# jts/nanopolish

Measured on NVIDIA H100. Metric: hmm_scored_events_per_sec, higher is better.
Workload: dtype f32

## Files before the change

nanopolish_b200/csrc/hmm_forward.cu:

```cuda
#include "hmm_forward_kernel.cuh"
#include <algorithm>
#include <cmath>
#include <vector>

using namespace nph_fwd;

namespace {

__global__ void read_prologue_kernel(const DevRead* __restrict__ reads, const double* __restrict__ drift,
                                     const float* __restrict__ ev_mean, const double* __restrict__ ev_time,
                                     float* __restrict__ level, uint32_t n_reads)
{
    for (uint32_t r = blockIdx.x; r < n_reads; r += gridDim.x) {
        const DevRead rd = reads[r];
        const double dr = drift[r];
        const float* m = ev_mean + rd.event_off;
        const double* t = ev_time + rd.event_off;
        float* out = level + rd.event_off;
        const double t0 = t[0];
        for (uint32_t i = threadIdx.x; i < rd.n_events; i += blockDim.x) {
            const float time = (float)__dsub_rn(t[i], t0);
            out[i] = (float)__dsub_rn((double)m[i], __dmul_rn((double)time, dr));
        }
    }
}

}

static void scratch_layout(const nph_ctx* ctx, NphArena& a, float4** params, float** edge)
{
    const size_t warps = (size_t)ctx->sm_count * kMaxWarpsPerCta;
    for (int si = 0; si < nph_ctx::kSideStreams; ++si) nph_wave_scratch(a, ctx->max_kpad, ctx->max_period, warps, &params[si], &edge[si]);
}

size_t nph_hmm_scratch_bytes(const nph_ctx* ctx)
{
    float4* params[nph_ctx::kSideStreams];
    float* edge[nph_ctx::kSideStreams];
    return nph_layout_bytes([&](NphArena& a) { scratch_layout(ctx, a, params, edge); });
}

int nph_launch_read_prologue(nph_ctx* ctx)
{
    const uint32_t n = (uint32_t)ctx->n_reads;
    if (n == 0) return NPH_OK;
    int grid = (int)std::min<size_t>(n, (size_t)ctx->sm_count * 16);
    read_prologue_kernel<<<grid, 256, 0, ctx->stream>>>(ctx->d_reads.p, ctx->d_drift.p, ctx->d_ev_mean.p,
                                                        ctx->d_ev_time.p, ctx->d_level.p, n);
    NPH_CUDA(ctx, cudaGetLastError());
    return NPH_OK;
}

int nph_launch_hmm_forward(nph_ctx* ctx, float* scores_dev)
{
    FwdParams p{};
    p.level = ctx->d_level.p;
    p.reads = ctx->d_reads.p;
    p.trans = ctx->d_trans.p;
    p.models = ctx->d_models.p;
    p.ranks = ctx->d_ranks.p;
    p.jobs = ctx->d_jobs.p;
    p.logsum_g = ctx->d_logsum.p;
    p.flank = ctx->d_flank.p;
    p.scores = scores_dev ? scores_dev : ctx->d_scores.p;
    p.kpad_stride = ctx->max_kpad;
    p.edge_stride = nph_edge_stride(ctx->max_period);
    p.c = ctx->consts;
    p.lsum_bias = NPH_LOGSUM_SAT_ADDR_BIAS;
    p.lsum_scale = 4u;
    p.progress = (ctx->levels_inflight && ctx->level_chunk_events) ? ctx->d_progress.p : nullptr;
    p.chunk_events = (uint32_t)ctx->level_chunk_events;
    float4* params[nph_ctx::kSideStreams];
    float* edge[nph_ctx::kSideStreams];
    NphArena scratch{ctx->d_scratch.p};
    scratch_layout(ctx, scratch, params, edge);

    NPH_CUDA(ctx, cudaMemsetAsync(ctx->d_counters.p, 0, sizeof(unsigned int) * NPH_NUM_COUNTERS, ctx->stream));
    NPH_CUDA(ctx, cudaEventRecord(ctx->ev0, ctx->stream));
    NPH_CUDA(ctx, cudaEventRecord(ctx->ev_fork, ctx->stream));
    std::vector<size_t> idx;
    for (size_t ci = 0; ci < ctx->classes.size(); ++ci) if (ctx->classes[ci].count) idx.push_back(ci);
    std::sort(idx.begin(), idx.end(), [&](size_t a, size_t b) { return ctx->classes[a].cost > ctx->classes[b].cost; });
    bool used[nph_ctx::kSideStreams] = {false, false, false, false};
    int launches = 0;
    for (size_t t = 0; t < idx.size(); ++t) {
        const size_t ci = idx[t];
        const auto& cl = ctx->classes[ci];
        const int si = (int)(t % nph_ctx::kSideStreams);
        cudaStream_t st = ctx->side[si];
        if (!used[si]) { NPH_CUDA(ctx, cudaStreamWaitEvent(st, ctx->ev_fork, 0)); used[si] = true; }
        p.scratch_params = params[si];
        p.scratch_edge = edge[si];
        int rc = NPH_ERR_STATE;
        switch (cl.group_width) {
            case 4: rc = launch_width<4, false>(ctx, p, cl, (int)ci, st); break;
            case 8: rc = launch_width<8, false>(ctx, p, cl, (int)ci, st); break;
            case 16: rc = launch_width<16, false>(ctx, p, cl, (int)ci, st); break;
            case 32: rc = cl.chained ? launch_width<32, true>(ctx, p, cl, (int)ci, st) : launch_width<32, false>(ctx, p, cl, (int)ci, st); break;
        }
        if (rc != NPH_OK) return rc;
        ++launches;
    }
    for (int si = 0; si < nph_ctx::kSideStreams; ++si) {
        if (!used[si]) continue;
        NPH_CUDA(ctx, cudaEventRecord(ctx->ev_join[si], ctx->side[si]));
        NPH_CUDA(ctx, cudaStreamWaitEvent(ctx->stream, ctx->ev_join[si], 0));
    }
    NPH_CUDA(ctx, cudaEventRecord(ctx->ev1, ctx->stream));
    nph_timing_events(ctx, launches);
    return NPH_OK;
}
```

nanopolish_b200/csrc/hmm_forward_kernel.cuh:

```cuda
#pragma once
#include "hmm_wavefront.cuh"
#include "exact_math.cuh"
#include <climits>

namespace nph_fwd {

static_assert(NPH_TBL_SMEM == NPH_LOGSUM_TBL_LEN, "the shared table must cover every index lsum_sat can form");

constexpr int kMaxWarpsPerCta = 24;
template <int C, int W> struct CtaShape { static constexpr int warps = (W == 32) ? 16 : (C <= 4 ? 24 : (C <= 6 ? 20 : 16)); };
constexpr unsigned kFull = 0xffffffffu;

struct FwdParams {
    const float* level;
    const DevRead* reads;
    const float2* trans;
    const DevModelView* models;
    const uint32_t* ranks;
    const nph_hmm_job* jobs;
    const uint32_t* order;
    uint32_t n_jobs;
    unsigned int* counter;
    const float* logsum_g;
    const float* flank;
    float* scores;
    float4* scratch_params;
    float* scratch_edge;
    uint32_t kpad_stride;
    uint32_t edge_stride;
    uint32_t lsum_bias;
    uint32_t lsum_scale;
    const uint32_t* progress;
    uint32_t chunk_events;
    HmmConsts c;
};

template <int C, int W, bool CHAIN>
__global__ void __launch_bounds__(CtaShape<C, W>::warps * 32, 1) hmm_forward_kernel(const FwdParams p)
{
    static_assert(W == 4 || W == 8 || W == 16 || W == 32, "group width");
    static_assert(!CHAIN || W == 32, "only full-warp groups chain strips");
    constexpr int G = 32 / W;
    constexpr int kWarpsPerCta = CtaShape<C, W>::warps;
    constexpr int kCtaThreads = kWarpsPerCta * 32;
    constexpr int STRIP = W * C;
    extern __shared__ float s_tbl[];
    for (int i = threadIdx.x; i < NPH_TBL_SMEM; i += kCtaThreads) s_tbl[i] = p.logsum_g[i];
    __syncthreads();
    const LogsumTable tb = make_logsum_table(s_tbl, p.lsum_bias, p.lsum_scale);

    const int lane = threadIdx.x & 31;
    const int gl = lane & (W - 1);
    const int grp = lane / W;
    const int warp_global = blockIdx.x * kWarpsPerCta + (threadIdx.x >> 5);
    float4* const my_params = warp_params(p.scratch_params, p.kpad_stride, warp_global) + (W < 32 ? grp * STRIP : 0);
    const EdgeRows edge = warp_edge_rows(p.scratch_edge, p.edge_stride, warp_global);

    const float NEG = -CUDART_INF_F;
    const float lp_mk = p.c.lp_mk, lp_mb = p.c.lp_mb, lp_bb = p.c.lp_bb, lp3 = p.c.lp_bk;
    const float lp_kk = p.c.lp_kk, lp_km = p.c.lp_km;

    for (;;) {
        const uint32_t base = nph_warp_pop(p.counter, (unsigned)G, lane);
        if (base >= p.n_jobs) break;
        const uint32_t slot = base + grp;
        const bool has_job = slot < p.n_jobs;
        const uint32_t job_idx = p.order[has_job ? slot : base];
        const nph_hmm_job job = p.jobs[job_idx];
        const DevRead rd = p.reads[job.read];
        const float2 tr = p.trans[job.read];
        const float lp_mm_self = tr.x, lp_mm_next = tr.y;
        const DevModelView mv = p.models[job.model_id];
        if (p.progress) {
            uint32_t need = has_job ? (uint32_t)((rd.event_off + rd.n_events - 1) / p.chunk_events) + 1u : 0u;
            need = __reduce_max_sync(kFull, need);
            if (lane == 0) {
                const volatile uint32_t* pr = p.progress;
                while (*pr < need) __nanosleep(500);
            }
            __syncwarp();
        }

        const nph_wave_geom geo = nph_wave_geometry((int)job.n_kmers, has_job ? nph_job_events(job) : 0, C, W, CHAIN);
        const int K = geo.K, E = geo.E, stride = job.stride, n_strips = geo.n_strips, P = geo.P;
        const bool pre_clip = (job.flags & NPH_HAF_ALLOW_PRE_CLIP) != 0;
        const bool post_clip = (job.flags & NPH_HAF_ALLOW_POST_CLIP) != 0;

        if (has_job) fill_job_gaussians<W>(my_params, mv, rd, p.ranks + job.rank_off, K, geo.kpad, gl, p.c.log_inv_sqrt_2pi);
        __syncwarp();

        const float* lv = p.level + rd.event_off;
        const long long e_first = (long long)job.event_start;
        const int last_strip = geo.last_strip(), end_lane = geo.end_lane(), end_slot = geo.end_slot();
        const int my_steps = has_job ? geo.total_steps() : 0;
        const int total_steps = (W == 32) ? my_steps : __reduce_max_sync(kFull, my_steps);
        const bool any_pre_clip = __any_sync(kFull, pre_clip);

        float mu[C], sd[C], cc[C], ry[C];
        float Mp[C], Bp[C], Kp[C], Tp[C];
#pragma unroll
        for (int c = 0; c < C; ++c) { mu[c] = 0.f; sd[c] = 1.f; cc[c] = 0.f; ry[c] = 1.f; Mp[c] = NEG; Bp[c] = NEG; Kp[c] = NEG; Tp[c] = NEG; }
        if (!CHAIN && gl * C < K) load_columns<C>(my_params, gl * C, mu, sd, cc, ry);
        float Lm_prev = NEG, Lt_prev = NEG, Lk_prev = NEG;
        float lp_end = NEG;
        int r = 1 - gl;
        int s = 0;
        float x_next = 0.f;
        if (r == 1 && E >= 1) x_next = lv[e_first];
        float em_next = NEG, et_next = NEG, ek_next = NEG;
        const long long x_step = (long long)stride * (long long)sizeof(float);
        unsigned long long x_addr = (unsigned long long)(lv + e_first) + (unsigned long long)((long long)r * x_step);
        const int end_row = (gl == end_lane) ? (post_clip ? 1 : E) : INT_MAX;

        for (int g = 0; g < total_steps; ++g) {
            float Lm = __shfl_up_sync(kFull, Mp[C - 1], 1, W);
            float Lt = __shfl_up_sync(kFull, Tp[C - 1], 1, W);
            float Lk = __shfl_up_sync(kFull, Kp[C - 1], 1, W);
            if (gl == 0) { Lm = CHAIN ? em_next : NEG; Lt = CHAIN ? et_next : NEG; Lk = CHAIN ? ek_next : NEG; }

            const bool in_strip = (r >= 1) && (!CHAIN || s < n_strips);
            const int col0 = (CHAIN ? s * STRIP : 0) + gl * C;
            const bool live = in_strip && (r <= E) && (col0 < K);
            const float x = x_next;

            if (CHAIN && in_strip && r == 1) {
#pragma unroll
                for (int c = 0; c < C; ++c) { Mp[c] = NEG; Bp[c] = NEG; Kp[c] = NEG; Tp[c] = NEG; }
                Lm_prev = NEG; Lt_prev = NEG; Lk_prev = NEG;
                if (col0 < K) load_columns<C>(my_params, col0, mu, sd, cc, ry);
            }
            {
                int rn = r + 1, sn = s;
                if (CHAIN && rn > P) { rn = 1; sn = s + 1; }
                if (rn >= 1 && rn <= E && (!CHAIN || sn < n_strips)) {
                    x_next = CHAIN ? lv[e_first + (long long)(rn - 1) * stride] : __ldca(reinterpret_cast<const float*>(x_addr));
                    if (CHAIN && gl == 0 && sn > 0) { em_next = edge.a[rn]; et_next = edge.b[rn]; ek_next = edge.c[rn]; }
                }
            }

            if (live) {
                const bool do_end = (!CHAIN || s == last_strip) && r >= end_row;

                float lm_prev = Lm_prev, lt_prev = Lt_prev, lk_prev = Lk_prev;
                float lm_cur = Lm, lt_cur = Lt, lk_cur = Lk;
                auto cell = [&](const int c, const bool with_soft) {
                    const float em = log_gauss(x, mu[c], sd[c], cc[c], ry[c]);
                    float m = __fadd_rn(lp_mm_self, Mp[c]);
                    m = lsum_sat(m, __fadd_rn(lp_mm_next, lm_prev), tb);
                    m = lsum_sat(m, Tp[c], tb);
                    m = lsum_sat(m, lt_prev, tb);
                    m = lsum_sat(m, __fadd_rn(lp_km, lk_prev), tb);
                    if (with_soft) m = lsum_sat(m, (col0 == 0 && (r == 1 || pre_clip)) ? p.flank[r - 1] : NEG, tb);
                    m = __fadd_rn(m, em);
                    const float b = lsum_sat(__fadd_rn(lp_mb, Mp[c]), __fadd_rn(lp_bb, Bp[c]), tb);
                    float kk = lsum_sat(__fadd_rn(lp_mk, lm_cur), lt_cur, tb);
                    kk = lsum_sat(kk, __fadd_rn(lp_kk, lk_cur), tb);
                    const float t = __fadd_rn(lp3, b);

                    lm_prev = Mp[c]; lt_prev = Tp[c]; lk_prev = Kp[c];
                    lm_cur = m; lt_cur = t; lk_cur = kk;
                    Mp[c] = m; Bp[c] = b; Kp[c] = kk; Tp[c] = t;
                };
                if (any_pre_clip || g == 0) cell(0, true);
                else cell(0, false);
#pragma unroll
                for (int c = 1; c < C; ++c) cell(c, false);
                Lm_prev = Lm; Lt_prev = Lt; Lk_prev = Lk;

                if (do_end) {
                    float Me = Mp[0], Be = Bp[0], Ke = Kp[0];
#pragma unroll
                    for (int c = 1; c < C; ++c) if (c == end_slot) { Me = Mp[c]; Be = Bp[c]; Ke = Kp[c]; }
                    const float post = p.flank[E - r];
                    lp_end = lsum_sat(lp_end, __fadd_rn(Me, post), tb);
                    lp_end = lsum_sat(lp_end, __fadd_rn(Be, post), tb);
                    lp_end = lsum_sat(lp_end, __fadd_rn(Ke, post), tb);
                }
                if (CHAIN && gl == W - 1 && s < last_strip) { edge.a[r] = Mp[C - 1]; edge.b[r] = Tp[C - 1]; edge.c[r] = Kp[C - 1]; }
            }

            r += 1;
            if (!CHAIN) x_addr += x_step;
            if (CHAIN && r > P) { r = 1; s += 1; }
            if (CHAIN && n_strips > 1) __syncwarp();
        }

        const float result = __shfl_sync(kFull, lp_end, (lane & ~(W - 1)) + end_lane);
        if (gl == 0 && has_job) p.scores[job_idx] = result;
        __syncwarp();
    }
}

template <int C, int W, bool CHAIN>
int launch_class(nph_ctx* ctx, const FwdParams& base, const nph_ctx::ClassLaunch& cl, int class_idx, cudaStream_t stream)
{
    FwdParams p = base;
    p.order = ctx->d_order.p + cl.first;
    p.n_jobs = (uint32_t)cl.count;
    p.counter = ctx->d_counters.p + class_idx;
    const size_t smem = sizeof(float) * NPH_TBL_SMEM;
    NPH_CUDA(ctx, cudaFuncSetAttribute(hmm_forward_kernel<C, W, CHAIN>, cudaFuncAttributeMaxDynamicSharedMemorySize, (int)smem));
    constexpr int kWarpsPerCta = CtaShape<C, W>::warps;
    int grid = ctx->sm_count;
    const size_t warps_needed = (cl.count + (32 / W) - 1) / (32 / W);
    if ((size_t)grid * kWarpsPerCta > warps_needed) grid = (int)((warps_needed + kWarpsPerCta - 1) / kWarpsPerCta);
    if (grid < 1) grid = 1;
    hmm_forward_kernel<C, W, CHAIN><<<grid, kWarpsPerCta * 32, smem, stream>>>(p);
    NPH_CUDA(ctx, cudaGetLastError());
    return NPH_OK;
}

template <int W, bool CHAIN> int launch_width(nph_ctx* ctx, const FwdParams& base, const nph_ctx::ClassLaunch& cl, int class_idx, cudaStream_t stream);

#define NPH_DEFINE_LAUNCH_WIDTH(W, CHAIN)                                                                              \
    template <> int launch_width<W, CHAIN>(nph_ctx * ctx, const FwdParams& base, const nph_ctx::ClassLaunch& cl, int class_idx, cudaStream_t stream) \
    {                                                                                                           \
        switch (cl.cols_per_lane) {                                                                             \
            case 1: return launch_class<1, W, CHAIN>(ctx, base, cl, class_idx, stream);                                       \
            case 2: return launch_class<2, W, CHAIN>(ctx, base, cl, class_idx, stream);                                       \
            case 3: return launch_class<3, W, CHAIN>(ctx, base, cl, class_idx, stream);                                       \
            case 4: return launch_class<4, W, CHAIN>(ctx, base, cl, class_idx, stream);                                       \
            case 5: return launch_class<5, W, CHAIN>(ctx, base, cl, class_idx, stream);                                       \
            case 6: return launch_class<6, W, CHAIN>(ctx, base, cl, class_idx, stream);                                       \
            case 7: return launch_class<7, W, CHAIN>(ctx, base, cl, class_idx, stream);                                       \
            case 8: return launch_class<8, W, CHAIN>(ctx, base, cl, class_idx, stream);                                       \
            case 9: return launch_class<9, W, CHAIN>(ctx, base, cl, class_idx, stream);                                       \
            case 10: return launch_class<10, W, CHAIN>(ctx, base, cl, class_idx, stream);                                     \
        }                                                                                                       \
        return NPH_ERR_STATE;                                                                                   \
    }

}
```

Measured before the change: 1.296 billion.

## Stream consecutive full-warp jobs through one wavefront to hide fill and drain

Adds a streaming path for full-warp, non-chained groups. When a job has more than 32 events and no clipping, the warp runs the jobs it pops back to back through a single skewed wavefront, so the next job's fill diagonal overlaps the previous job's drain. Per-warp job descriptors are double-buffered in shared memory and Gaussian parameters in two scratch lines, which is why the params stride grows. The aim is to remove the idle lanes during each job's ramp-up and ramp-down. In exchange the kernel gains complexity, register pressure and more shared and scratch memory.

```diff
diff --git a/nanopolish_b200/csrc/hmm_forward.cu b/nanopolish_b200/csrc/hmm_forward.cu
--- a/nanopolish_b200/csrc/hmm_forward.cu
+++ b/nanopolish_b200/csrc/hmm_forward.cu
@@ -27,10 +27,12 @@
 
 }
 
+static uint32_t params_stride(const nph_ctx* ctx) { return ctx->max_kpad + 32 * NPH_MAX_COLS; }
+
 static void scratch_layout(const nph_ctx* ctx, NphArena& a, float4** params, float** edge)
 {
     const size_t warps = (size_t)ctx->sm_count * kMaxWarpsPerCta;
-    for (int si = 0; si < nph_ctx::kSideStreams; ++si) nph_wave_scratch(a, ctx->max_kpad, ctx->max_period, warps, &params[si], &edge[si]);
+    for (int si = 0; si < nph_ctx::kSideStreams; ++si) nph_wave_scratch(a, params_stride(ctx), ctx->max_period, warps, &params[si], &edge[si]);
 }
 
 size_t nph_hmm_scratch_bytes(const nph_ctx* ctx)
@@ -63,7 +65,7 @@
     p.logsum_g = ctx->d_logsum.p;
     p.flank = ctx->d_flank.p;
     p.scores = scores_dev ? scores_dev : ctx->d_scores.p;
-    p.kpad_stride = ctx->max_kpad;
+    p.kpad_stride = params_stride(ctx);
     p.edge_stride = nph_edge_stride(ctx->max_period);
     p.c = ctx->consts;
     p.lsum_bias = NPH_LOGSUM_SAT_ADDR_BIAS;
diff --git a/nanopolish_b200/csrc/hmm_forward_kernel.cuh b/nanopolish_b200/csrc/hmm_forward_kernel.cuh
--- a/nanopolish_b200/csrc/hmm_forward_kernel.cuh
+++ b/nanopolish_b200/csrc/hmm_forward_kernel.cuh
@@ -35,6 +35,184 @@
     HmmConsts c;
 };
 
+template <int C, class SoftFn>
+__device__ __forceinline__ void row_update(const float x, const float (&mu)[C], const float (&sd)[C], const float (&cc)[C], const float (&ry)[C],
+                                           float (&Mp)[C], float (&Bp)[C], float (&Kp)[C], float (&Tp)[C],
+                                           float lm_prev, float lt_prev, float lk_prev, float lm_cur, float lt_cur, float lk_cur,
+                                           const float lp_mm_self, const float lp_mm_next, const HmmConsts& k, const bool with_soft, const SoftFn& soft,
+                                           const LogsumTable& tb)
+{
+    auto cell = [&](const int c, const bool fold_soft) {
+        const float em = log_gauss(x, mu[c], sd[c], cc[c], ry[c]);
+        float m = __fadd_rn(lp_mm_self, Mp[c]);
+        m = lsum_sat(m, __fadd_rn(lp_mm_next, lm_prev), tb);
+        m = lsum_sat(m, Tp[c], tb);
+        m = lsum_sat(m, lt_prev, tb);
+        m = lsum_sat(m, __fadd_rn(k.lp_km, lk_prev), tb);
+        if (fold_soft) m = lsum_sat(m, soft(), tb);
+        m = __fadd_rn(m, em);
+        const float b = lsum_sat(__fadd_rn(k.lp_mb, Mp[c]), __fadd_rn(k.lp_bb, Bp[c]), tb);
+        float kk = lsum_sat(__fadd_rn(k.lp_mk, lm_cur), lt_cur, tb);
+        kk = lsum_sat(kk, __fadd_rn(k.lp_kk, lk_cur), tb);
+        const float t = __fadd_rn(k.lp_bk, b);
+
+        lm_prev = Mp[c]; lt_prev = Tp[c]; lk_prev = Kp[c];
+        lm_cur = m; lt_cur = t; lk_cur = kk;
+        Mp[c] = m; Bp[c] = b; Kp[c] = kk; Tp[c] = t;
+    };
+    if (with_soft) cell(0, true);
+    else cell(0, false);
+#pragma unroll
+    for (int c = 1; c < C; ++c) cell(c, false);
+}
+
+template <int C>
+__device__ __forceinline__ float end_fold(float lp_end, const float (&Mp)[C], const float (&Bp)[C], const float (&Kp)[C], const int end_slot, const float post,
+                                          const LogsumTable& tb)
+{
+    float Me = Mp[0], Be = Bp[0], Ke = Kp[0];
+#pragma unroll
+    for (int c = 1; c < C; ++c) if (c == end_slot) { Me = Mp[c]; Be = Bp[c]; Ke = Kp[c]; }
+    lp_end = lsum_sat(lp_end, __fadd_rn(Me, post), tb);
+    lp_end = lsum_sat(lp_end, __fadd_rn(Be, post), tb);
+    return lsum_sat(lp_end, __fadd_rn(Ke, post), tb);
+}
+
+struct JobIn { nph_hmm_job job; DevRead rd; float2 tr; DevModelView mv; };
+__device__ __forceinline__ JobIn fetch_job(const FwdParams& p, const uint32_t job_idx, const bool has_job, const int lane)
+{
+    JobIn j;
+    j.job = p.jobs[job_idx];
+    j.rd = p.reads[j.job.read];
+    j.tr = p.trans[j.job.read];
+    j.mv = p.models[j.job.model_id];
+    if (p.progress) {
+        uint32_t need = has_job ? (uint32_t)((j.rd.event_off + j.rd.n_events - 1) / p.chunk_events) + 1u : 0u;
+        need = __reduce_max_sync(kFull, need);
+        if (lane == 0) {
+            const volatile uint32_t* pr = p.progress;
+            while (*pr < need) __nanosleep(500);
+        }
+        __syncwarp();
+    }
+    return j;
+}
+
+__device__ __forceinline__ bool streams(const nph_hmm_job& job, const int E)
+{
+    return E > 32 && (job.flags & (NPH_HAF_ALLOW_PRE_CLIP | NPH_HAF_ALLOW_POST_CLIP)) == 0;
+}
+
+struct StreamJob {
+    unsigned long long x_addr;
+    uint32_t idx;
+    int E, end_lane, end_slot;
+    float lp_mm_self, lp_mm_next;
+    int x_step;
+};
+
+template <int C>
+__device__ __forceinline__ int stream_job(const FwdParams& p, float4* params, const uint32_t job_idx, const JobIn& j, const int lane, StreamJob* s)
+{
+    const nph_wave_geom geo = nph_wave_geometry((int)j.job.n_kmers, nph_job_events(j.job), C, 32, false);
+    if (lane == 0) {
+        s->x_addr = (unsigned long long)(p.level + j.rd.event_off + j.job.event_start);
+        s->idx = job_idx;
+        s->E = geo.E; s->end_lane = geo.end_lane(); s->end_slot = geo.end_slot();
+        s->lp_mm_self = j.tr.x; s->lp_mm_next = j.tr.y;
+        s->x_step = j.job.stride * (int)sizeof(float);
+    }
+    fill_job_gaussians<32>(params, j.mv, j.rd, p.ranks + j.job.rank_off, geo.K, geo.kpad, lane, p.c.log_inv_sqrt_2pi);
+    return geo.E;
+}
+
+template <int C>
+__device__ uint32_t run_stream(const FwdParams& p, const LogsumTable& tb, const HmmConsts& k, float4* params, int lane, const uint32_t job_idx,
+                               const JobIn& first)
+{
+    asm volatile("" : "+l"(params), "+r"(lane));
+    __shared__ StreamJob s_jobs[CtaShape<C, 32>::warps][2];
+    volatile StreamJob* const sj = s_jobs[threadIdx.x >> 5];
+    auto line = [&](const int i) { return params + (i & 1) * (32 * C); };
+    int n = 0;
+    int E = stream_job<C>(p, line(0), job_idx, first, lane, const_cast<StreamJob*>(&sj[0]));
+
+    const float NEG = -CUDART_INF_F;
+    float mu[C], sd[C], cc[C], ry[C];
+    float Mp[C], Bp[C], Kp[C], Tp[C];
+#pragma unroll
+    for (int c = 0; c < C; ++c) { mu[c] = 0.f; sd[c] = 1.f; cc[c] = 0.f; ry[c] = 1.f; Mp[c] = NEG; Bp[c] = NEG; Kp[c] = NEG; Tp[c] = NEG; }
+    float Lm_prev = NEG, Lt_prev = NEG, Lk_prev = NEG;
+    float lp_mm_self = 0.f, lp_mm_next = 0.f;
+    unsigned long long x_addr = 0;
+    int x_step = 0;
+    float x_next = 0.f;
+    bool has_a = false, has_b = true;
+    uint32_t ended_by = p.n_jobs;
+    __syncwarp();
+    for (;;) {
+        volatile StreamJob& a = sj[(n + 1) & 1];
+        volatile StreamJob& b = sj[n & 1];
+        const int window = has_b ? 33 : a.end_lane + 1;
+        for (int t = 0; t < window; ++t) {
+            float Lm = __shfl_up_sync(kFull, Mp[C - 1], 1);
+            float Lt = __shfl_up_sync(kFull, Tp[C - 1], 1);
+            float Lk = __shfl_up_sync(kFull, Kp[C - 1], 1);
+            if (lane == 0) { Lm = NEG; Lt = NEG; Lk = NEG; }
+            const float x = x_next;
+            if (has_b && t == lane + 1) {
+#pragma unroll
+                for (int c = 0; c < C; ++c) { Mp[c] = NEG; Bp[c] = NEG; Kp[c] = NEG; Tp[c] = NEG; }
+                Lm_prev = NEG; Lt_prev = NEG; Lk_prev = NEG;
+                load_columns<C>(line(n), lane * C, mu, sd, cc, ry);
+                lp_mm_self = b.lp_mm_self; lp_mm_next = b.lp_mm_next;
+            }
+            if (t == lane) { x_addr = b.x_addr; x_step = b.x_step; }
+            if (t < lane ? has_a : has_b) {
+                x_next = __ldca(reinterpret_cast<const float*>(x_addr));
+                x_addr += x_step;
+            }
+            if (t <= lane ? has_a : has_b) {
+                row_update<C>(x, mu, sd, cc, ry, Mp, Bp, Kp, Tp, Lm_prev, Lt_prev, Lk_prev, Lm, Lt, Lk, lp_mm_self, lp_mm_next, k, true,
+                              [&] { return (lane == 0 && t == 1) ? p.flank[0] : NEG; }, tb);
+                Lm_prev = Lm; Lt_prev = Lt; Lk_prev = Lk;
+                if (t == lane && lane == a.end_lane) p.scores[a.idx] = end_fold<C>(NEG, Mp, Bp, Kp, a.end_slot, p.flank[0], tb);
+            }
+        }
+        if (!has_b) break;
+
+#pragma unroll 1
+        for (int g = E - 33; g > 0; --g) {
+            float Lm = __shfl_up_sync(kFull, Mp[C - 1], 1);
+            float Lt = __shfl_up_sync(kFull, Tp[C - 1], 1);
+            float Lk = __shfl_up_sync(kFull, Kp[C - 1], 1);
+            if (lane == 0) { Lm = NEG; Lt = NEG; Lk = NEG; }
+            const float x = x_next;
+            x_next = __ldca(reinterpret_cast<const float*>(x_addr));
+            x_addr += x_step;
+            row_update<C>(x, mu, sd, cc, ry, Mp, Bp, Kp, Tp, Lm_prev, Lt_prev, Lk_prev, Lm, Lt, Lk, lp_mm_self, lp_mm_next, k, false,
+                          [&] { return NEG; }, tb);
+            Lm_prev = Lm; Lt_prev = Lt; Lk_prev = Lk;
+        }
+        has_a = true;
+
+        __syncwarp();
+        has_b = false;
+        const uint32_t slot = nph_warp_pop(p.counter, 1u, lane);
+        if (slot < p.n_jobs) {
+            const uint32_t n_idx = p.order[slot];
+            const JobIn j = fetch_job(p, n_idx, true, lane);
+            has_b = streams(j.job, nph_job_events(j.job));
+            if (has_b) E = stream_job<C>(p, line(n + 1), n_idx, j, lane, const_cast<StreamJob*>(&sj[(n + 1) & 1]));
+            else ended_by = slot;
+        }
+        load_columns<C>(line(n), lane * C, mu, sd, cc, ry);
+        n += 1;
+        __syncwarp();
+    }
+    return ended_by;
+}
+
 template <int C, int W, bool CHAIN>
 __global__ void __launch_bounds__(CtaShape<C, W>::warps * 32, 1) hmm_forward_kernel(const FwdParams p)
 {
@@ -57,32 +235,27 @@
     const EdgeRows edge = warp_edge_rows(p.scratch_edge, p.edge_stride, warp_global);
 
     const float NEG = -CUDART_INF_F;
-    const float lp_mk = p.c.lp_mk, lp_mb = p.c.lp_mb, lp_bb = p.c.lp_bb, lp3 = p.c.lp_bk;
-    const float lp_kk = p.c.lp_kk, lp_km = p.c.lp_km;
-
+    const HmmConsts& k = p.c;
+
+    uint32_t ended_stream = UINT_MAX;
     for (;;) {
-        const uint32_t base = nph_warp_pop(p.counter, (unsigned)G, lane);
+        const uint32_t base = ended_stream != UINT_MAX ? ended_stream : nph_warp_pop(p.counter, (unsigned)G, lane);
+        ended_stream = UINT_MAX;
         if (base >= p.n_jobs) break;
         const uint32_t slot = base + grp;
         const bool has_job = slot < p.n_jobs;
         const uint32_t job_idx = p.order[has_job ? slot : base];
-        const nph_hmm_job job = p.jobs[job_idx];
-        const DevRead rd = p.reads[job.read];
-        const float2 tr = p.trans[job.read];
-        const float lp_mm_self = tr.x, lp_mm_next = tr.y;
-        const DevModelView mv = p.models[job.model_id];
-        if (p.progress) {
-            uint32_t need = has_job ? (uint32_t)((rd.event_off + rd.n_events - 1) / p.chunk_events) + 1u : 0u;
-            need = __reduce_max_sync(kFull, need);
-            if (lane == 0) {
-                const volatile uint32_t* pr = p.progress;
-                while (*pr < need) __nanosleep(500);
-            }
-            __syncwarp();
-        }
+        const JobIn ji = fetch_job(p, job_idx, has_job, lane);
+        const nph_hmm_job& job = ji.job;
+        const DevRead& rd = ji.rd;
+        const DevModelView& mv = ji.mv;
+        const float lp_mm_self = ji.tr.x, lp_mm_next = ji.tr.y;
 
         const nph_wave_geom geo = nph_wave_geometry((int)job.n_kmers, has_job ? nph_job_events(job) : 0, C, W, CHAIN);
         const int K = geo.K, E = geo.E, stride = job.stride, n_strips = geo.n_strips, P = geo.P;
+        if constexpr (W == 32 && !CHAIN) {
+            if (streams(job, E)) { ended_stream = run_stream<C>(p, tb, k, my_params, lane, job_idx, ji); continue; }
+        }
         const bool pre_clip = (job.flags & NPH_HAF_ALLOW_PRE_CLIP) != 0;
         const bool post_clip = (job.flags & NPH_HAF_ALLOW_POST_CLIP) != 0;
 
@@ -141,41 +314,11 @@
             if (live) {
                 const bool do_end = (!CHAIN || s == last_strip) && r >= end_row;
 
-                float lm_prev = Lm_prev, lt_prev = Lt_prev, lk_prev = Lk_prev;
-                float lm_cur = Lm, lt_cur = Lt, lk_cur = Lk;
-                auto cell = [&](const int c, const bool with_soft) {
-                    const float em = log_gauss(x, mu[c], sd[c], cc[c], ry[c]);
-                    float m = __fadd_rn(lp_mm_self, Mp[c]);
-                    m = lsum_sat(m, __fadd_rn(lp_mm_next, lm_prev), tb);
-                    m = lsum_sat(m, Tp[c], tb);
-                    m = lsum_sat(m, lt_prev, tb);
-                    m = lsum_sat(m, __fadd_rn(lp_km, lk_prev), tb);
-                    if (with_soft) m = lsum_sat(m, (col0 == 0 && (r == 1 || pre_clip)) ? p.flank[r - 1] : NEG, tb);
-                    m = __fadd_rn(m, em);
-                    const float b = lsum_sat(__fadd_rn(lp_mb, Mp[c]), __fadd_rn(lp_bb, Bp[c]), tb);
-                    float kk = lsum_sat(__fadd_rn(lp_mk, lm_cur), lt_cur, tb);
-                    kk = lsum_sat(kk, __fadd_rn(lp_kk, lk_cur), tb);
-                    const float t = __fadd_rn(lp3, b);
-
-                    lm_prev = Mp[c]; lt_prev = Tp[c]; lk_prev = Kp[c];
-                    lm_cur = m; lt_cur = t; lk_cur = kk;
-                    Mp[c] = m; Bp[c] = b; Kp[c] = kk; Tp[c] = t;
-                };
-                if (any_pre_clip || g == 0) cell(0, true);
-                else cell(0, false);
-#pragma unroll
-                for (int c = 1; c < C; ++c) cell(c, false);
+                row_update<C>(x, mu, sd, cc, ry, Mp, Bp, Kp, Tp, Lm_prev, Lt_prev, Lk_prev, Lm, Lt, Lk, lp_mm_self, lp_mm_next, k, any_pre_clip || g == 0,
+                              [&] { return (col0 == 0 && (r == 1 || pre_clip)) ? p.flank[r - 1] : NEG; }, tb);
                 Lm_prev = Lm; Lt_prev = Lt; Lk_prev = Lk;
 
-                if (do_end) {
-                    float Me = Mp[0], Be = Bp[0], Ke = Kp[0];
-#pragma unroll
-                    for (int c = 1; c < C; ++c) if (c == end_slot) { Me = Mp[c]; Be = Bp[c]; Ke = Kp[c]; }
-                    const float post = p.flank[E - r];
-                    lp_end = lsum_sat(lp_end, __fadd_rn(Me, post), tb);
-                    lp_end = lsum_sat(lp_end, __fadd_rn(Be, post), tb);
-                    lp_end = lsum_sat(lp_end, __fadd_rn(Ke, post), tb);
-                }
+                if (do_end) lp_end = end_fold<C>(lp_end, Mp, Bp, Kp, end_slot, p.flank[E - r], tb);
                 if (CHAIN && gl == W - 1 && s < last_strip) { edge.a[r] = Mp[C - 1]; edge.b[r] = Tp[C - 1]; edge.c[r] = Kp[C - 1]; }
             }
 
```

Result: faster. 1.353 billion, median of 6 (+4.4%).
